# goroda/GPEXP

Measured on AMD Instinct MI355X. Metric: GP-fit+IVAR-eval points/s at N=32768 d=8 (wall-time in ms_per_step); value = (N+M)/t_step, SURVEY 8d's N/t_fit and M/t_IVAR are points_per_s_fit / points_per_s_ivar right behind it, higher is better.
Workload: dtype f64; 1 GPU; C4: N=32768 d=8 Matern-5/2 (rho=0.5,s=1,noise=0.1) kfill+potrf+potrs+logdet+IVAR over M=32768 MC points; N=32768, d=8, M=32768, kernel=matern52, seed=32768, parallelism=1 GPU

## Files before the change

### gpexp_amd/_lib.py

```python
import ctypes as C
import os

import numpy as np

_HERE = os.path.dirname(os.path.abspath(__file__))
LIB_PATH = os.path.join(_HERE, "libgpx_hip.so")

c_i64 = C.c_int64
c_dp = C.POINTER(C.c_double)
c_ip = C.POINTER(c_i64)
c_vp = C.c_void_p

_SIGS = {
    "gpx_abi_version": (C.c_int, []),
    "gpx_last_error": (C.c_char_p, []),
    "gpx_create": (C.c_int, [C.c_int, C.POINTER(c_vp)]),
    "gpx_destroy": (C.c_int, [c_vp]),
    "gpx_sync": (C.c_int, [c_vp]),
    "gpx_trim": (C.c_int, [c_vp]),
    "gpx_device_info": (C.c_int, [c_vp, C.c_char_p, C.c_int, C.POINTER(C.c_int), c_ip, C.POINTER(C.c_int)]),
    "gpx_mat_from_host": (C.c_int, [c_vp, c_dp, c_i64, c_i64, C.c_int, C.POINTER(c_vp)]),
    "gpx_mat_alloc": (C.c_int, [c_vp, c_i64, c_i64, C.c_int, C.POINTER(c_vp)]),
    "gpx_mat_free": (C.c_int, [c_vp, c_vp]),
    "gpx_mat_clone": (C.c_int, [c_vp, c_vp, C.POINTER(c_vp)]),
# ... 95 lines not shown
    "gpx_points_set_box": (C.c_int, [c_vp, c_vp, c_dp, c_dp, C.c_int]),
    "gpx_dist2_panel_pack": (C.c_int, [c_vp, c_vp, c_i64, c_i64, c_i64, c_i64, c_vp, c_i64, c_i64]),
    "gpx_dist2_diag_pack": (C.c_int, [c_vp, c_vp, c_i64, c_i64, c_i64, c_vp, c_i64, c_i64]),
    "gpx_dist2_update": (C.c_int, [c_vp, c_vp, c_i64, c_i64, c_i64, c_i64, c_vp, c_i64, c_i64, c_i64, c_i64]),
    "gpx_dist2_update_multi": (C.c_int, [c_vp, c_vp, c_i64, c_i64, c_i64, c_i64, c_i64, C.c_int, C.c_int, C.c_int, C.c_int, c_i64,
                                         C.c_int, C.POINTER(c_vp), c_ip, C.c_int]),
    "gpx_dist2_pack_rows": (C.c_int, [c_vp, c_vp, c_i64, c_i64, c_i64, c_vp, c_i64, c_i64, c_i64, c_i64]),
    "gpx_dist2_pack_diag": (C.c_int, [c_vp, c_vp, c_i64, c_i64, c_i64, c_vp, c_i64]),
    "gpx_program_run": (C.c_int, [c_vp, c_ip, c_i64, c_ip, c_i64, c_dp]),
    "gpx_program_capture": (C.c_int, [c_vp, c_ip, c_i64, c_ip, c_i64, C.POINTER(c_vp)]),
    "gpx_graph_launch": (C.c_int, [c_vp, c_vp, c_dp, c_ip]),
    "gpx_graph_free": (C.c_int, [c_vp, c_vp]),
    "gpx_dist2_unpack_rows": (C.c_int, [c_vp, c_vp, c_i64, c_i64, c_i64, c_i64, c_vp, c_i64, c_i64, c_i64]),
    "gpx_dist2_unpack_diag": (C.c_int, [c_vp, c_vp, c_i64, c_i64, c_i64, c_vp, c_i64]),
    "gpx_dist2_unpack_diag_at": (C.c_int, [c_vp, c_vp, c_i64, c_i64, c_i64, c_vp, c_i64, c_i64]),
    "gpx_dist2_trsv_diag": (C.c_int, [c_vp, c_vp, c_i64, c_i64, c_i64, c_vp, c_i64, C.c_int]),
    "gpx_dist2_gemv": (C.c_int, [c_vp, c_vp, c_i64, c_i64, c_i64, c_i64, c_vp, c_i64, c_vp, c_i64, C.c_int]),
    "gpx_dist2_logdet_acc": (C.c_int, [c_vp, c_vp, c_i64, c_i64, c_i64, c_i64, c_vp]),
    "gpx_stream_select": (C.c_int, [c_vp, C.c_int]),
    "gpx_event_record": (C.c_int, [c_vp, C.c_int]),
    "gpx_event_wait": (C.c_int, [c_vp, C.c_int]),
    "gpx_dist_finish": (C.c_int, [c_vp, c_vp]),
    "gpx_ivar_grad": (C.c_int, [c_vp, C.c_int, C.c_int, c_dp, C.c_int, c_vp, c_vp, c_vp, c_dp, c_dp]),
    "gpx_ivar_grad_w": (C.c_int, [c_vp, C.c_int, C.c_int, c_dp, C.c_int, c_vp, c_vp, c_vp, c_dp, c_vp, c_dp]),
    "gpx_ivar_grad_rows": (C.c_int, [c_vp, C.c_int, C.c_int, c_dp, C.c_int, c_vp, c_vp, c_vp, c_vp, c_i64, c_dp]),
    "gpx_var_grad": (C.c_int, [c_vp, C.c_int, C.c_int, c_dp, C.c_int, c_vp, c_vp, c_vp, c_dp, c_dp, c_dp, c_dp]),
    "gpx_var_grad_newpt": (C.c_int, [c_vp, C.c_int, C.c_int, c_dp, C.c_int, c_vp, c_vp, c_vp, c_dp]),
    "gpx_fitc_var_grad": (C.c_int, [c_vp, c_vp, C.c_int, C.c_int, c_dp, C.c_int, c_vp, c_vp, c_dp, c_dp, c_dp, c_dp]),
    "gpx_fitc_var_grad_newpt": (C.c_int, [c_vp, c_vp, C.c_int, C.c_int, c_dp, C.c_int, c_vp, c_vp, c_dp]),
    "gpx_profile_enable": (C.c_int, [c_vp, C.c_int]),
    "gpx_profile_reset": (C.c_int, [c_vp]),
    "gpx_profile_get": (C.c_int, [c_vp, C.c_int, c_ip, c_dp, c_dp, c_dp]),
    "gpx_dbg_gemm": (C.c_int, [c_vp, c_vp, c_vp, c_vp, C.c_int, C.c_int, C.c_int]),
    "gpx_dbg_gemm_tri": (C.c_int, [c_vp, c_vp, c_vp, c_vp, C.c_int, C.c_int, C.c_int]),
    "gpx_dbg_gemm_ksplit": (C.c_int, [c_vp, c_vp, c_vp, c_vp, C.c_int, C.c_int]),
    "gpx_dbg_kfill_plan": (C.c_int, [c_vp, C.c_int, C.c_int, c_dp, C.c_int, c_vp, c_vp, C.POINTER(C.c_int), c_dp]),
    "gpx_dbg_colreduce_plan": (C.c_int, [c_i64, c_i64, C.POINTER(c_i64), C.POINTER(c_i64)]),
    "gpx_dbg_panel_bcast_plan": (C.c_int, [C.c_int, C.c_int, c_i64, C.c_int, C.POINTER(c_i64), C.POINTER(C.c_int),
                                           C.POINTER(c_i64), c_i64, C.POINTER(c_i64)]),
    "gpx_dbg_guard_violations": (c_i64, [c_vp]),
    "gpx_dbg_guard_selftest": (C.c_int, [c_vp]),
    "gpx_dbg_spin": (C.c_int, [c_vp, C.c_int]),
    "gpx_dbg_spin_us": (C.c_int, [c_vp, c_i64]),
    "gpx_dbg_stamp": (C.c_int, [c_vp, C.c_int]),
    "gpx_dbg_spin_until": (C.c_int, [c_vp, C.c_int, c_i64]),
    "gpx_dbg_event_elapsed": (C.c_int, [c_vp, C.c_int, C.c_int, c_dp]),
    "gpx_dbg_leaf_stamps": (C.c_int, [c_vp, c_vp, C.c_int, C.POINTER(c_i64)]),
}

_lib = None


def load():
    global _lib
    if _lib is not None:
        return _lib
    path = os.environ.get("GPX_LIB_PATH", LIB_PATH)
    if not os.path.exists(path):
        raise ImportError(
            "gpexp_amd: %s not found - the HIP library is required (no CPU fallback). "
            "Build it with `make -C gpexp_amd/csrc` or __graft_entry__.build()." % path)
    lib = C.CDLL(path)
    for name, (res, args) in _SIGS.items():
        fn = getattr(lib, name)
        fn.restype = res
        fn.argtypes = args
# ... 41 lines not shown
```

### gpexp_amd/csrc/api.hip

```cpp
#include "gpx_internal.h"
#include <stdarg.h>
#include <stdio.h>
#include <string.h>
#include <math.h>
#include <stdlib.h>

static thread_local char g_err[1024] = "";

void gpx_set_error(const char* fmt, ...) {
  va_list ap;
  va_start(ap, fmt);
  vsnprintf(g_err, sizeof(g_err), fmt, ap);
  va_end(ap);
}

static constexpr int64_t GUARD = 4096;

int gpx_dev_alloc(gpx_ctx* ctx, int64_t bytes, void** out) {
  if (bytes <= 0) bytes = 8;
  bytes = gpx_round_up(bytes, 256);
  const int64_t key = bytes + (ctx->guard ? 2 * GUARD : 0);
  void* base = nullptr;
  auto it = ctx->pool.find(key);
  if (it != ctx->pool.end()) {
// ... 1383 lines not shown
  KParams kp;
  GPX_TRY(gpx_make_kparams(kind, d, hyp, nhyp, &kp));
  GPX_TRY(gpx_kparams_sets(ctx, &kp, X, Z));
  *exact = kp.exact;
  for (int k = 0; k < d; ++k) center[k] = kp.center[k];
  return 0;
}

int gpx_dbg_gemm_ksplit(gpx_ctx* ctx, const gpx_mat* A, const gpx_mat* B, gpx_mat* C, int mode, int parts) {
  GPX_ARG(ctx && A && B && C && mode >= 0 && mode <= 3 && parts > 0, "bad argument");
  const int64_t m = C->prows, n = C->pcols, k = A->pcols;
  GPX_ARG(A->prows == m && B->prows == n && B->pcols == k, "operand shapes");
  void* P;
  const int64_t pb = (int64_t)parts * m * n * 8;
  GPX_TRY(gpx_dev_alloc(ctx, pb, &P));
  int r = mode <= 1 ? launch_gemm_ksplit(ctx, A->p, A->ld, B->p, B->ld, C->p, C->ld, m, n, k, mode == 1, parts, (double*)P)
                    : launch_gemm_ksplit_small(ctx, A->p, A->ld, B->p, B->ld, C->p, C->ld, m, n, k, mode == 3, parts, (double*)P);
  (void)hipStreamSynchronize(ctx->stream);
  gpx_dev_release(ctx, P, pb);
  return r;
}

int gpx_dbg_gemm(gpx_ctx* ctx, const gpx_mat* A, const gpx_mat* B, gpx_mat* C, int bt, int accumulate, int lower) {
  GPX_ARG(ctx && A && B && C, "NULL argument");
  const int64_t m = C->prows, n = C->pcols, k = A->pcols;
  GPX_ARG(A->prows == m, "A rows");
  GPX_ARG(bt ? (B->prows == n && B->pcols == k) : (B->prows == k && B->pcols == n), "B shape");
  GPX_TRY(launch_gemm(ctx, A->p, A->ld, B->p, B->ld, C->p, C->ld, m, n, k, bt != 0, accumulate != 0,
                      lower != 0));
  GPX_HIP(hipStreamSynchronize(ctx->stream));
  return 0;
}

}
```

### gpexp_amd/csrc/chol.hip

```cpp
#include "gpx_internal.h"
#include <math.h>
#include <stdlib.h>
#include <stddef.h>

namespace {

constexpr int NB = GPX_TILE;
constexpr int LS = NB + 1;

typedef double d4 __attribute__((ext_vector_type(4)));

__device__ __forceinline__ double readlane_d(double v, int srclane) {
  int lo = __builtin_amdgcn_readlane(__double2loint(v), srclane);
  int hi = __builtin_amdgcn_readlane(__double2hiint(v), srclane);
  return __hiloint2double(hi, lo);
}

constexpr int LB = 16;
constexpr int TS17 = LB + 1;
constexpr int BSZ = LB * TS17;
constexpr int LEAF_CB = LB * LB + 64 + LB;

__device__ __forceinline__ constexpr int sb_off(int I, int J) { return (I * (I + 1) / 2 + J) * BSZ; }

// ... 1166 lines not shown

int chol_binv_ensure(gpx_ctx* ctx, gpx_mat* Lm) {
  const int64_t n = Lm->prows, ib = potrs_block(n);
  if (Lm->binv && Lm->binv_ib == ib) return 0;
  const int64_t nblk = (n + ib - 1) / ib;
  const int64_t bytes = chol_binv_elems(n) * 8;
  if (Lm->binv && Lm->binv_bytes != bytes) {
    gpx_dev_release(ctx, Lm->binv, Lm->binv_bytes);
    Lm->binv = nullptr;
  }
  if (!Lm->binv) {
    void* p;
    GPX_TRY(gpx_dev_alloc(ctx, bytes, &p));
    Lm->binv = (double*)p;
    Lm->binv_bytes = bytes;
  }
  void* pt;
  GPX_TRY(gpx_dev_alloc(ctx, nblk * ib * ib * 8, &pt));
  int r = binv_build_range(ctx, Lm->p, Lm->ld, Lm->aux, Lm->binv, ib, n, (double*)pt);
  if (r == 0) r = chol_binv_finish(ctx, Lm, ib);
  (void)hipStreamSynchronize(ctx->stream);
  gpx_dev_release(ctx, pt, nblk * ib * ib * 8);
  if (r != 0) Lm->binv_ib = 0;
  return r;
}

struct PotrsPlan {
  const double* L;
  int64_t ld, n, ib, nblk;
  int64_t sib;
  const double* binv;
  const double* binvT;
  double* part;
};
static inline int64_t blk_off(const PotrsPlan& P, int64_t b) { return b * P.ib < P.n ? b * P.ib : P.n; }
static inline const double* blk_inv(const PotrsPlan& P, const double* base, int64_t b) {
  const int64_t row = b * P.ib, sb = row / P.sib, within = row - sb * P.sib;
  return base + sb * P.sib * P.sib + within * P.sib + within;
}

static int potrs_fwd(gpx_ctx* ctx, const PotrsPlan& P, int64_t b0, int64_t b1, double* rhs, double* x) {
  if (b1 - b0 == 1) {
    const int64_t o = blk_off(P, b0), sz = blk_off(P, b0 + 1) - o;
    hipLaunchKernelGGL(binv_gemv_kernel, dim3((unsigned)((sz + 3) / 4)), dim3(256), 0, ctx->stream, blk_inv(P, P.binv, b0),
                       P.sib, sz, rhs + o, x + o, 1);
    return 0;
  }
  const int64_t mid = (b0 + b1) / 2;
  GPX_TRY(potrs_fwd(ctx, P, b0, mid, rhs, x));
  const int64_t r0 = blk_off(P, mid), r1 = blk_off(P, b1), c0 = blk_off(P, b0);
  int64_t wg = (r1 - r0 + 3) / 4;
  if (wg > 4096) wg = 4096;
  hipLaunchKernelGGL(gemv_sub_kernel, dim3((unsigned)wg), dim3(256), 0, ctx->stream, P.L + r0 * P.ld + c0, P.ld, r1 - r0, r0 - c0,
                     x + c0, rhs + r0);
  return potrs_fwd(ctx, P, mid, b1, rhs, x);
}

static int potrs_bwd(gpx_ctx* ctx, const PotrsPlan& P, int64_t b0, int64_t b1, double* rhs, double* z) {
  if (b1 - b0 == 1) {
    const int64_t o = blk_off(P, b0), sz = blk_off(P, b0 + 1) - o;
    hipLaunchKernelGGL(binv_gemv_kernel, dim3((unsigned)((sz + 3) / 4)), dim3(256), 0, ctx->stream, blk_inv(P, P.binvT, b0),
                       P.sib, sz, rhs + o, z + o, 0);
    return 0;
  }
  const int64_t mid = (b0 + b1) / 2;
  GPX_TRY(potrs_bwd(ctx, P, mid, b1, rhs, z));
  const int64_t r0 = blk_off(P, mid), r1 = blk_off(P, b1), c0 = blk_off(P, b0);
  GPX_TRY(launch_colreduce(ctx, P.L + r0 * P.ld + c0, P.ld, r1 - r0, r0 - c0, z + r0, rhs + c0, P.part, 1));
  return potrs_bwd(ctx, P, b0, mid, rhs, z);
}

static int trsm_left_oop_rec(gpx_ctx* ctx, const PotrsPlan& P, int64_t b0, int64_t b1, double* B, int64_t ldb, double* W,
                             int64_t ldw, int64_t m) {
  if (b1 - b0 == 1) {
    const int64_t o = blk_off(P, b0), sz = blk_off(P, b0 + 1) - o;
    return launch_gemm_tri(ctx, blk_inv(P, P.binv, b0), P.sib, B + o * ldb, ldb, W + o * ldw, ldw, sz, m, sz, false, false,
                           false, 1);
  }
  const int64_t mid = (b0 + b1) / 2;
  GPX_TRY(trsm_left_oop_rec(ctx, P, b0, mid, B, ldb, W, ldw, m));
  const int64_t r0 = blk_off(P, mid), r1 = blk_off(P, b1), c0 = blk_off(P, b0);
  GPX_TRY(launch_gemm(ctx, P.L + r0 * P.ld + c0, P.ld, W + c0 * ldw, ldw, B + r0 * ldb, ldb, r1 - r0, m, r0 - c0, false, true,
                      false));
  return trsm_left_oop_rec(ctx, P, mid, b1, B, ldb, W, ldw, m);
}

int chol_trsm_left_oop(gpx_ctx* ctx, gpx_mat* Lm, double* B, int64_t ldb, double* W, int64_t ldw, int64_t m) {
  GPX_ARG(Lm && Lm->factored && Lm->aux && B && W && B != W, "trsm: matrix has not been factored / bad buffers");
  if (m == 0) return 0;
  GPX_TRY(chol_binv_ensure(ctx, Lm));
  PotrsPlan P;
  P.L = Lm->p;
  P.ld = Lm->ld;
  P.n = Lm->prows;
  P.sib = Lm->binv_ib;
  P.ib = P.sib < 1024 ? P.sib : 1024;
  P.nblk = (P.n + P.ib - 1) / P.ib;
  P.binv = Lm->binv;
  P.binvT = nullptr;
  P.part = nullptr;
  return trsm_left_oop_rec(ctx, P, 0, P.nblk, B, ldb, W, ldw, m);
}

int chol_trsm_left_group(gpx_ctx* ctx, const double* Lg, int64_t ld, const double* invd, int64_t w, int64_t below, int64_t ib,
                         double* B, int64_t ldb, int64_t m, double* inv, double* tmp, double* W, int64_t ldw) {
  GPX_ARG(Lg && invd && B && inv && tmp && W && W != B && w > 0 && w % NB == 0 && ib >= NB && ib % NB == 0, "trsm group: bad arguments");
  if (m == 0) return 0;
  GPX_TRY(binv_build_range(ctx, Lg, ld, invd, inv, ib, w, tmp));
  PotrsPlan P;
  P.L = Lg;
  P.ld = ld;
  P.n = w;
  P.ib = P.sib = ib;
  P.nblk = (w + ib - 1) / ib;
  P.binv = inv;
  P.binvT = nullptr;
  P.part = nullptr;
  GPX_TRY(trsm_left_oop_rec(ctx, P, 0, P.nblk, B, ldb, W, ldw, m));
  if (below > 0) GPX_TRY(launch_gemm(ctx, Lg + w * ld, ld, W, ldw, B + w * ldb, ldb, below, m, w, false, true, false));
  return gpx_copy2d(ctx, W, ldw, B, ldb, w, m);
}

int64_t chol_potrs_scratch_bytes(int64_t n) { return n * 8 + colreduce_partial_elems(n, n) * 8 + 64; }

int chol_potrs(gpx_ctx* ctx, gpx_mat* Lm, double* v, double* scratch) {
  GPX_ARG(Lm && Lm->factored && Lm->aux && v && scratch, "potrs: matrix has not been factored / NULL vector");
  GPX_ARG(Lm->ld % 2 == 0, "potrs: leading dimension must be even");
  GPX_TRY(chol_binv_ensure(ctx, Lm));
  PotrsPlan P;
  P.L = Lm->p;
  P.ld = Lm->ld;
  P.n = Lm->prows;
  P.ib = P.sib = Lm->binv_ib;
  P.nblk = (P.n + P.ib - 1) / P.ib;
// ... 53 lines not shown
```

### gpexp_amd/csrc/gemm_f64.hip

```cpp
#include "gpx_internal.h"
#include <stdlib.h>

namespace {

typedef double d4 __attribute__((ext_vector_type(4)));

constexpr int KB = 16;
constexpr int SA = KB + 1;

template <bool BT, int TE>
struct Smem {
  double a[2][TE * SA];
  double b[2][BT ? TE * SA : KB * (TE + 16)];
};

template <bool LOWER>
__device__ __forceinline__ bool tile_of(int sblk, int within, int tiles_m, int tiles_n, int sb_cols, int sb_shift,
                                        int* by, int* bx, int rot = 0) {
  const int sbm = (1 << sb_shift) - 1;
  int sr, sc;
  if (LOWER) {
    const int nsr = (tiles_m + sbm) >> sb_shift;
    const int noff = nsr * (nsr - 1) / 2;
    if (sblk < noff) {
// ... 7 lines not shown
  } else {
    sr = sblk / sb_cols;
    sc = sblk - sr * sb_cols;
    if (rot) {
      if ((8 % sb_cols) == 0)
        sc = (sc + (sblk >> 3)) % sb_cols;
      else if ((sb_cols & 7) == 0)
        sc = (sc + sr) % sb_cols;
    }
  }
  *by = (sr << sb_shift) + (within >> sb_shift);
  *bx = (sc << sb_shift) + (within & sbm);
  if (!LOWER && rot == 2) {
    *by = (sr << sb_shift) + (within & sbm);
    *bx = (sc << sb_shift) + (sbm - (within >> sb_shift));
  }
  if (!LOWER && rot == 4) {
    *by = (sr << sb_shift) + (sbm - (within >> sb_shift));
    *bx = (sc << sb_shift) + (within & sbm);
  }
  if (!LOWER && rot == 3) {
    *by = (sr << sb_shift) + (within & sbm);
    *bx = (sc << sb_shift) + (within >> sb_shift);
  }
  if (*by >= tiles_m || *bx >= tiles_n) return false;
  if (LOWER && *bx > *by) return false;
  return true;
}

struct NoSeg {
  static constexpr bool on = false;
};

template <bool BT, bool ACC, int TE, class SEGF = NoSeg>
__device__ __forceinline__ void gemm_tile(Smem<BT, TE>& sm, const double* A, int64_t lda, const double* B, int64_t ldb,
                                          double* C, int64_t ldc, int nk, int by, int bx, const SEGF& segf = SEGF()) {
  constexpr int SBN = TE + 16;
  constexpr int FI = TE / 32;
  constexpr int NL = TE / 32;
  constexpr int WS = TE / 2;
  constexpr int BKR = 512 / TE;
  constexpr int A_BUF = TE * SA;
  constexpr int B_BUF = BT ? TE * SA : KB * SBN;

  const int t = threadIdx.x;
  const int lane = t & 63, wave = t >> 6;
  const int wm = wave >> 1, wn = wave & 1;
  const int64_t m0 = (int64_t)by * TE, n0 = (int64_t)bx * TE;

  const int ar = t >> 3, ac = (t & 7) * 2;
  const int br = t / (TE / 2), bc = (t % (TE / 2)) * 2;
  const unsigned voff_a = (unsigned)((ar * lda + ac) * 8);
  const unsigned voff_b = BT ? (unsigned)((ar * ldb + ac) * 8) : (unsigned)((br * ldb + bc) * 8);
  const char* const Abase = reinterpret_cast<const char*>(A + m0 * lda);
  const char* const Bbase = reinterpret_cast<const char*>(BT ? (B + n0 * ldb) : (B + n0));
  const int64_t a_rs = 32 * lda * 8;
  const int64_t b_rs = (BT ? 32 * ldb : BKR * ldb) * 8;
  const int64_t a_ks = (int64_t)KB * 8;
  const int64_t b_ks = (BT ? (int64_t)KB : (int64_t)KB * ldb) * 8;

  double2 Pa0, Pa1, Pa2, Pa3, Pb0, Pb1, Pb2, Pb3;
  const int64_t b_rs2 = 2 * b_rs, b_rs3 = 3 * b_rs, a_rs2 = 2 * a_rs, a_rs3 = 3 * a_rs;
#define GPX_LD16(base_, voff_) (*reinterpret_cast<const double2*>((base_) + (voff_)))
#define GPX_GLOAD_AT(S_, ap_, bp_)                                                                    \
  do {                                                                                                \
    S_##a0 = GPX_LD16(ap_, voff_a);                                                                    \
    S_##a1 = GPX_LD16(ap_ + a_rs, voff_a);                                                             \
    if (NL == 4) {                                                                                    \
      S_##a2 = GPX_LD16(ap_ + a_rs2, voff_a);                                                          \
// ... 140 lines not shown
      GPX_MFMAS(1);
      GPX_MFMAS(2);
      GPX_PIN();
      GPX_SSTORE(P, buf ^ 1);
      __syncthreads();
      GPX_PIN();
      GPX_FRAGS(buf ^ 1, 0, 0);
      GPX_FRAGS(buf ^ 1, 1, 1);
      GPX_FRAGS(buf ^ 1, 2, 2);
      GPX_PIN();
      GPX_MFMAS(3);
      GPX_FRAGS(buf ^ 1, 3, 3);
    }
    }
    GPX_MFMAS(0);
    GPX_MFMAS(1);
    GPX_MFMAS(2);
    GPX_MFMAS(3);
#undef GPX_STEP
#undef GPX_FRAGS
#undef GPX_MFMAS
#undef GPX_PIN
#undef GPX_PIN_ALL
  }
#undef GPX_GLOAD
#undef GPX_GLOAD_AT
#undef GPX_LD16
#undef GPX_SSTORE
#undef GPX_ST2
#undef GPX_STB
#undef GPX_COMPUTE

  double* Cw = C + (m0 + wm * WS + fk) * ldc + n0 + wn * WS + fr;
#pragma unroll
  for (int i = 0; i < FI; ++i)
#pragma unroll
    for (int v = 0; v < 4; ++v) {
      double* cp = Cw + (int64_t)(i * 16 + 4 * v) * ldc;
      if (ACC) {
        double cv[FI];
#pragma unroll
        for (int j = 0; j < FI; ++j) cv[j] = cp[j * 16];
#pragma unroll
        for (int j = 0; j < FI; ++j) cp[j * 16] = cv[j] - acc[i][j][v];
      } else {
#pragma unroll
        for (int j = 0; j < FI; ++j) cp[j * 16] = acc[i][j][v];
      }
    }
}

template <bool BT, bool ACC, bool LOWER, int TE, int TRI>
__global__ __launch_bounds__(256, 2) void gemm_f64_kernel(const double* A, int64_t lda, const double* B, int64_t ldb,
                                                          double* C, int64_t ldc, int nk, int tiles_m, int tiles_n,
                                                          int sb_cols, int sb_shift, int main_wgs, int tail_m0,
                                                          int tail_tn) {
  constexpr int tri = TRI;
  __shared__ Smem<BT, TE> sm;
  if (TE == 64 && tail_tn < 0) __builtin_amdgcn_s_setprio(3);
  const int w = blockIdx.x;
  if (TE == 128 && w >= main_wgs) {
    const int wt = w - main_wgs;
    const int by = wt / tail_tn, bx = wt - by * tail_tn;
    if (LOWER && 64 * bx > tail_m0 + 64 * by + 63) return;
    int64_t k0 = 0;
    if (tri == 3) k0 = tail_m0 + 64 * by;
    gemm_tile<BT, ACC, 64>(reinterpret_cast<Smem<BT, 64>&>(sm), A + (int64_t)tail_m0 * lda + k0, lda, B + k0, ldb,
                                 C + (int64_t)tail_m0 * ldc, ldc, nk - (int)(k0 / KB), by, bx);
    return;
  }
  const int xcd = w & 7, q = w >> 3;
  const int sbs2 = 2 * sb_shift;
  int by, bx;
  if (!tile_of<LOWER>((q >> sbs2) * 8 + xcd, q & ((1 << sbs2) - 1), tiles_m, tiles_n, sb_cols, sb_shift, &by, &bx,
                      tri == 2 ? 2 : (tri == 4 ? 3 : (tri == 1 ? 4 : 0))))
    return;
  int nkt = nk;
  if (tri == 1) nkt = min(nk, (by + 1) * (TE / KB));
  if (tri == 2) nkt = min(nk, (bx + 1) * (TE / KB));
  if (tri == 3) {
    const int64_t k0 = (int64_t)by * TE;
    A += k0;
    B += k0;
    nkt = nk - by * (TE / KB);
  }
  if (tri == 4) {
    const int64_t k0 = (int64_t)bx * TE;
    A += k0;
    B += k0 * ldb;
    nkt = nk - bx * (TE / KB);
  }
  gemm_tile<BT, ACC, TE>(sm, A, lda, B, ldb, C, ldc, nkt, by, bx);
}

template <bool BT, bool ACC>
__global__ __launch_bounds__(256, 2) void gemm_f64_batched_kernel(const double* A, int64_t lda, int64_t sa,
                                                                  const double* B, int64_t ldb, int64_t sb, double* C,
                                                                  int64_t ldc, int64_t sc, int nk, int tiles_n, int hiprio) {
  __shared__ Smem<BT, 64> sm;
  if (hiprio) __builtin_amdgcn_s_setprio(3);
  const int64_t b = blockIdx.y;
  const int by = blockIdx.x / tiles_n, bx = blockIdx.x - by * tiles_n;
  gemm_tile<BT, ACC, 64>(sm, A + b * sa, lda, B + b * sb, ldb, C + b * sc, ldc, nk, by, bx);
}

template <bool LOWER>
__global__ __launch_bounds__(256, 2) void gemm_f64_ksplit_kernel(const double* A, int64_t lda, const double* B, int64_t ldb,
                                                                 double* P, int64_t n, int64_t sp, int nk_slice, int parts,
                                                                 int tiles_m, int tiles_n, int sb_cols, int sb_shift) {
  __shared__ Smem<true, 128> sm;
  const int w = blockIdx.x, xcd = w & 7, q = w >> 3, sbs2 = 2 * sb_shift;
  const int job = (q >> sbs2) * 8 + xcd, within = q & ((1 << sbs2) - 1);
  int sb, slice;
  if (LOWER) {
    const int nsr = (tiles_m + (1 << sb_shift) - 1) >> sb_shift, noff = nsr * (nsr - 1) / 2;
    if (job < parts * noff) {
      slice = job / noff;
      sb = job - slice * noff;
    } else {
      const int jj = job - parts * noff;
      slice = jj / nsr;
      sb = noff + jj - slice * nsr;
    }
  } else {
    const int nsb = ((tiles_m + (1 << sb_shift) - 1) >> sb_shift) * sb_cols;
// ... 223 lines not shown
      gpx_set_error("gemm: triangular-operand mode %d is not instantiated for bt=%d accumulate=%d", tri, (int)bt, (int)accumulate);
      return -1;
    }
#undef GPX_GT
    GPX_HIP(hipGetLastError());
    return 0;
  }
#define GPX_K(BT_, ACC_, LOW_, TE_) GPX_KT(BT_, ACC_, LOW_, TE_, 0)
#define GPX_G(BT_, ACC_, LOW_)          \
  do {                                  \
    if (te == 64)                       \
      GPX_K(BT_, ACC_, LOW_, 64);       \
    else                                \
      GPX_K(BT_, ACC_, LOW_, 128);      \
  } while (0)
  if (bt) {
    if (accumulate) {
      if (lower) GPX_G(true, true, true); else GPX_G(true, true, false);
    } else {
      if (lower) GPX_G(true, false, true); else GPX_G(true, false, false);
    }
  } else {
    if (accumulate) {
      if (lower) GPX_G(false, true, true); else GPX_G(false, true, false);
    } else {
      if (lower) GPX_G(false, false, true); else GPX_G(false, false, false);
    }
  }
#undef GPX_G
#undef GPX_K
#undef GPX_KT
  GPX_HIP(hipGetLastError());
  return 0;
}

int launch_dist2_update(gpx_ctx* ctx, double* C, int64_t ldc, int64_t lr0, int64_t m, int64_t lc0, int64_t n, int64_t nb, int Pr,
                        int Pc, int pr, int pc, int64_t piece_stride, int64_t dsz, int nseg, const double* const* g,
                        const int64_t* ks, int below_diag) {
  if (m == 0 || n == 0 || nseg == 0) return 0;
  GPX_ARG(nseg > 0 && nseg <= GPX_SEG_MAX && Pr >= 1 && Pr <= GPX_MAX_PR && Pc >= 1, "dist2 update: too many segments / grid rows");
  GPX_ARG(m % 128 == 0 && n % 128 == 0 && nb % 128 == 0 && lr0 % nb == 0 && lc0 % nb == 0 && (ldc % 2) == 0, "dist2 update: alignment");
  Dist2Upd u;
  for (int s = 0; s < nseg; ++s) {
    u.g[s] = g[s];
    for (int p = 0; p < Pr; ++p) u.li0[s][p] = (int)(ks[s] + 1 <= p ? 0 : (ks[s] - p) / Pr + 1);
  }
  u.nseg = nseg;
  u.seg_nk = (int)(nb / KB);
  u.Pr = Pr; u.Pc = Pc; u.pr = pr; u.pc = pc;
  u.nb = (int)nb;
  u.gld = (int)gpx_g_ld(nb);
  u.li_first = (int)(lr0 / nb);
  u.lj_first = (int)(lc0 / nb);
  u.below_diag = below_diag;
  u.piece_stride = piece_stride;
  u.dsz = dsz;
  double tiles128 = 0.0;
  for (int64_t lj = lc0 / nb; lj * nb < lc0 + n; ++lj) {
    const int64_t J = lj * Pc + pc;
    const int64_t cw = (lc0 + n - lj * nb) < nb ? (lc0 + n - lj * nb) : nb;
    for (int64_t li = lr0 / nb; li * nb < lr0 + m; ++li) {
      const int64_t I = li * Pr + pr;
      if (I < J || (below_diag && I == J)) continue;
      const int64_t rh = (lr0 + m - li * nb) < nb ? (lr0 + m - li * nb) : nb;
      tiles128 += (double)(rh / 128) * (double)(cw / 128);
    }
// ... 51 lines not shown
```

### gpexp_amd/csrc/gpx_internal.h

```cpp
#pragma once
#include <hip/hip_runtime.h>
#include <stdint.h>
#include <stdlib.h>
#include <string>
#include <vector>
#include <map>
#include <memory>
#include <unordered_set>
#include "../../include/gpx.h"
#include "../../include/gpx_dist.h"
#include "../../include/gpx_debug.h"

#define GPX_TILE 128
#define GPX_MAXD GPX_MAX_DIM
#define GPX_NSTREAMS 6
#define GPX_SEG_MAX 8
#ifndef GPX_G_SKEW
#define GPX_G_SKEW 0
#endif
#define GPX_MAX_PR 4

void gpx_set_error(const char* fmt, ...);
#define GPX_HIP(call)                                                                   \
  do {                                                                                  \
// ... 128 lines not shown
  do {                            \
    if ((d_) <= 1) { CALL(1); }   \
    else if ((d_) <= 2) { CALL(2); } \
    else if ((d_) <= 4) { CALL(4); } \
    else if ((d_) <= 8) { CALL(8); } \
    else if ((d_) <= 16) { CALL(16); } \
    else { CALL(32); }            \
  } while (0)

extern "C" int64_t gpx_eval_chunk(int64_t np);

int launch_kfill(gpx_ctx* ctx, const KParams& kp, const double* A, int64_t na, const double* B, int64_t nb,
                 int symmetric, const double* d_nugget, int64_t nugget_len, double nugget_scalar,
                 double* out, int64_t prows, int64_t pcols, int64_t ld);
int launch_kfill_offset(gpx_ctx* ctx, const KParams& kp, const double* X, int64_t n, int64_t row_off, int64_t col_off,
                        const double* d_nugget, int64_t nugget_len, double nugget_scalar, double* out, int64_t prows,
                        int64_t pcols, int64_t ld);
int launch_kdiag(gpx_ctx* ctx, const KParams& kp, const double* Z, int64_t m, double* out);
int launch_kfill_cyclic(gpx_ctx* ctx, const KParams& kp, const double* X, int64_t n, const double* d_nugget,
                        int64_t nugget_len, double nugget_scalar, double* out, int64_t prows, int64_t pcols, int64_t ld,
                        int64_t nb, int Pr, int pr, int Pc, int pc);
int gpx_copy2d(gpx_ctx* ctx, const double* src, int64_t lds_, double* dst, int64_t ldd, int64_t rows, int64_t cols);
int gpx_copy2d_lower(gpx_ctx* ctx, const double* src, int64_t lds_, double* dst, int64_t ldd, int64_t n);
int launch_kfill_rows(gpx_ctx* ctx, const KParams& kp, const double* X, int64_t n, int64_t row0, const double* d_nugget,
                      int64_t nugget_len, double nugget_scalar, double* out, int64_t prows_band, int64_t pcols,
                      int64_t ld);

static inline int gpx_chain_prio(const gpx_ctx* ctx) { return ctx->stream == ctx->streams[1] ? 1 : 0; }
int launch_gemm(gpx_ctx* ctx, const double* A, int64_t lda, const double* B, int64_t ldb, double* C, int64_t ldc,
                int64_t m, int64_t n, int64_t k, bool bt, bool accumulate, bool lower);

int launch_gemm_tri(gpx_ctx* ctx, const double* A, int64_t lda, const double* B, int64_t ldb, double* C, int64_t ldc,
                    int64_t m, int64_t n, int64_t k, bool bt, bool accumulate, bool lower, int tri);
int launch_gemm_ksplit(gpx_ctx* ctx, const double* A, int64_t lda, const double* B, int64_t ldb, double* C, int64_t ldc,
                       int64_t m, int64_t n, int64_t k, bool lower, int64_t parts, double* P, bool assign = false);
int launch_gemm_ksplit_small(gpx_ctx* ctx, const double* A, int64_t lda, const double* B, int64_t ldb, double* C, int64_t ldc,
                             int64_t m, int64_t n, int64_t k, bool assign, int64_t parts, double* P);
int launch_gemm_batched(gpx_ctx* ctx, const double* A, int64_t lda, int64_t sa, const double* B, int64_t ldb, int64_t sb,
                        double* C, int64_t ldc, int64_t sc, int64_t m, int64_t n, int64_t k, bool bt, bool accumulate,
                        int64_t batch);

int launch_dist2_update(gpx_ctx* ctx, double* C, int64_t ldc, int64_t lr0, int64_t m, int64_t lc0, int64_t n, int64_t nb, int Pr,
                        int Pc, int pr, int pc, int64_t piece_stride, int64_t dsz, int nseg, const double* const* g,
                        const int64_t* ks, int below_diag);

int launch_leaf(gpx_ctx* ctx, double* A, int64_t ld, double* inv, int64_t base_index, int64_t n_valid);
int chol_potrf(gpx_ctx* ctx, double* A, int64_t ld, int64_t n, double* invd, int64_t n_valid);
int chol_potrf_nozero(gpx_ctx* ctx, double* A, int64_t ld, int64_t n, double* invd, int64_t base, int64_t n_valid);
int chol_trsm_right(gpx_ctx* ctx, const double* L, int64_t ldl, const double* invd, double* X, int64_t ldx,
                    int64_t m, int64_t n);
int chol_trsm_right_n(gpx_ctx* ctx, const double* L, int64_t ldl, const double* invd, double* X, int64_t ldx,
                      int64_t m, int64_t n);
int chol_trsm_left(gpx_ctx* ctx, const double* L, int64_t ldl, const double* invd, double* B, int64_t ldb,
                   int64_t n, int64_t m);
int chol_trsv(gpx_ctx* ctx, const double* L, int64_t ld, const double* invd, double* y, int64_t n, bool transposed);
int64_t chol_trsv_scratch_bytes(int64_t n);
int chol_trsv_with_scratch(gpx_ctx* ctx, const double* L, int64_t ld, const double* invd, double* y, int64_t n,
                           bool transposed, double* scratch);
int launch_logdet(gpx_ctx* ctx, const double* L, int64_t ld, int64_t n, double* d_out);
int chol_trtri(gpx_ctx* ctx, const gpx_mat* L, double* Linv, double* tmp);
int chol_binv_ensure(gpx_ctx* ctx, gpx_mat* L);
int chol_trsm_right_trailing(gpx_ctx* ctx, gpx_mat* L, int64_t r0, double* X, int64_t ldx, int64_t m, int transposed, double* T);
int chol_trsm_right_leading(gpx_ctx* ctx, gpx_mat* L, int64_t ncols, double* X, int64_t ldx, int64_t m, double* T, int64_t tcap);
int chol_trsm_right_n_leading(gpx_ctx* ctx, gpx_mat* L, int64_t ncols, double* X, int64_t ldx, int64_t m, double* T);
int chol_block_inverse(gpx_ctx* ctx, const double* D, int64_t ldd, const double* invd, double* inv, int64_t w, double* tmp);
int64_t chol_binv_order(int64_t n);
// ... 28 lines not shown
```

### gpexp_amd/device.py

```python
import ctypes as C
import atexit
import os

import numpy as np

from . import _lib
from ._lib import check, as_f64, dptr, c_vp, c_i64, GpxError

K_SE, K_MATERN32, K_MATERN52, K_MEHLER = 0, 1, 2, 3
PROF_CLASSES = ["kfill", "gemm", "leaf", "trsv", "reduce", "greedy", "comm", "kcross"]

_ctx = None


class Context:

    def __init__(self, device=None):
        self.lib = _lib.load()
        if device is None:
            device = int(os.environ.get("LOCAL_RANK", "0"))
        h = c_vp()
        rc = self.lib.gpx_create(int(device), C.byref(h))
        if rc != 0:
            raise RuntimeError("gpexp_amd needs an MI355X: " + self.lib.gpx_last_error().decode())
# ... 617 lines not shown

def var_grad(ctx, spec, L, X, Z, noise_deriv=None, eval_bias=None, dk_bias=None):
    out = np.empty((X.shape[0] * spec.d, Z.shape[0]))
    nd = as_f64(noise_deriv) if noise_deriv is not None else None
    eb = as_f64(eval_bias) if eval_bias is not None else None
    db = as_f64(dk_bias) if dk_bias is not None else None
    check(ctx.lib.gpx_var_grad(ctx.h, *spec.args(), L.h, X.h, Z.h, dptr(nd), dptr(eb), dptr(db), dptr(out)))
    return out


def var_grad_newpt(ctx, spec, L, X, Z):
    out = np.empty(Z.shape[0] * spec.d)
    check(ctx.lib.gpx_var_grad_newpt(ctx.h, *spec.args(), L.h, X.h, Z.h, dptr(out)))
    return out


def kfill_plan(ctx, spec, X, Z=None):
    ex = C.c_int()
    cen = np.zeros(spec.d)
    check(ctx.lib.gpx_dbg_kfill_plan(ctx.h, *spec.args(), X.h, Z.h if Z is not None else None, C.byref(ex), dptr(cen)))
    return bool(ex.value), cen


def dbg_gemm_tri(ctx, A, B, Cm, bt, accumulate, tri):
    check(ctx.lib.gpx_dbg_gemm_tri(ctx.h, A.h, B.h, Cm.h, int(bt), int(accumulate), int(tri)))


def dbg_gemm_ksplit(ctx, A, B, Cm, mode, parts):
    check(ctx.lib.gpx_dbg_gemm_ksplit(ctx.h, A.h, B.h, Cm.h, int(mode), int(parts)))


def dbg_gemm(ctx, A, B, Cm, bt, accumulate, lower=False):
    check(ctx.lib.gpx_dbg_gemm(ctx.h, A.h, B.h, Cm.h, int(bt), int(accumulate), int(lower)))
```

### include/gpx_debug.h

```cpp
#ifndef GPX_DEBUG_H
#define GPX_DEBUG_H
#include "gpx.h"
#ifdef __cplusplus
extern "C" {
#endif

int gpx_dbg_gemm(gpx_ctx* ctx, const gpx_mat* A, const gpx_mat* B, gpx_mat* C, int bt, int accumulate, int lower);
int gpx_dbg_gemm_tri(gpx_ctx* ctx, const gpx_mat* A, const gpx_mat* B, gpx_mat* C, int bt, int accumulate, int tri);
int gpx_dbg_gemm_ksplit(gpx_ctx* ctx, const gpx_mat* A, const gpx_mat* B, gpx_mat* C, int mode, int parts);
int gpx_dbg_spin(gpx_ctx* ctx, int ms);
int64_t gpx_dbg_guard_violations(gpx_ctx* ctx);
int gpx_dbg_guard_selftest(gpx_ctx* ctx);
int gpx_dbg_panel_bcast_plan(int W, int me, int64_t small_elems, int npieces, const int64_t* counts, const int* roots,
                             int64_t* ops, int64_t max_ops, int64_t* nops);
int gpx_dbg_colreduce_plan(int64_t rows, int64_t pcols, int64_t* nchunk, int64_t* bound_elems);
int gpx_dbg_kfill_plan(gpx_ctx* ctx, int kind, int d, const double* hyp, int nhyp, const gpx_mat* X, const gpx_mat* Z,
                       int* exact, double* center);

int gpx_dbg_spin_us(gpx_ctx* ctx, int64_t us);
int gpx_dbg_stamp(gpx_ctx* ctx, int slot);
int gpx_dbg_spin_until(gpx_ctx* ctx, int slot, int64_t us);
int gpx_dbg_event_elapsed(gpx_ctx* ctx, int id0, int id1, double* ms);

int gpx_dbg_leaf_stamps(gpx_ctx* ctx, gpx_mat* K, int fast, int64_t* out30);

#ifdef __cplusplus
}
#endif
#endif
```

Before: 97150 points/s.

## Use one-level Strassen for large GEMM updates in left out-of-place TRSM

Adds a one-level Strassen GEMM path for the trailing updates inside the recursive left triangular solve, used when the update block is large (at least 8192 rows and inner dimension, 4096 columns). Operand sums are formed by a small elementwise kernel. Five of the seven half-size products use a new dual-destination epilogue that subtracts into two C quadrants at once, so no temporary product buffers are needed. The aim is to cut roughly one eighth of the FP64 multiply work in the dominant solve GEMMs. The costs are extra scratch memory, extra memory traffic for the sums and the read-modify-write of two outputs, and slightly weaker numerical error bounds. It can be turned off with GPX_STRASSEN=0.

```diff
diff --git a/gpexp_amd/_lib.py b/gpexp_amd/_lib.py
--- a/gpexp_amd/_lib.py
+++ b/gpexp_amd/_lib.py
@@ -151,6 +151,7 @@
     "gpx_profile_reset": (C.c_int, [c_vp]),
     "gpx_profile_get": (C.c_int, [c_vp, C.c_int, c_ip, c_dp, c_dp, c_dp]),
     "gpx_dbg_gemm": (C.c_int, [c_vp, c_vp, c_vp, c_vp, C.c_int, C.c_int, C.c_int]),
+    "gpx_dbg_gemm_strassen": (C.c_int, [c_vp, c_vp, c_vp, c_vp]),
     "gpx_dbg_gemm_tri": (C.c_int, [c_vp, c_vp, c_vp, c_vp, C.c_int, C.c_int, C.c_int]),
     "gpx_dbg_gemm_ksplit": (C.c_int, [c_vp, c_vp, c_vp, c_vp, C.c_int, C.c_int]),
     "gpx_dbg_kfill_plan": (C.c_int, [c_vp, C.c_int, C.c_int, c_dp, C.c_int, c_vp, c_vp, C.POINTER(C.c_int), c_dp]),
diff --git a/gpexp_amd/csrc/api.hip b/gpexp_amd/csrc/api.hip
--- a/gpexp_amd/csrc/api.hip
+++ b/gpexp_amd/csrc/api.hip
@@ -1439,4 +1439,13 @@
   return 0;
 }
 
-}
+int gpx_dbg_gemm_strassen(gpx_ctx* ctx, const gpx_mat* A, const gpx_mat* B, gpx_mat* C) {
+  GPX_ARG(ctx && A && B && C, "NULL argument");
+  const int64_t m = C->prows, n = C->pcols, k = A->pcols;
+  GPX_ARG(A->prows == m && B->prows == k && B->pcols == n, "operand shapes");
+  GPX_TRY(launch_gemm_strassen(ctx, A->p, A->ld, B->p, B->ld, C->p, C->ld, m, n, k, nullptr, 0));
+  GPX_HIP(hipStreamSynchronize(ctx->stream));
+  return 0;
+}
+
+}
diff --git a/gpexp_amd/csrc/chol.hip b/gpexp_amd/csrc/chol.hip
--- a/gpexp_amd/csrc/chol.hip
+++ b/gpexp_amd/csrc/chol.hip
@@ -1222,6 +1222,9 @@
   const double* binv;
   const double* binvT;
   double* part;
+  bool strassen = false;
+  double* sscr = nullptr;
+  int64_t sscr_bytes = 0;
 };
 static inline int64_t blk_off(const PotrsPlan& P, int64_t b) { return b * P.ib < P.n ? b * P.ib : P.n; }
 static inline const double* blk_inv(const PotrsPlan& P, const double* base, int64_t b) {
@@ -1260,6 +1263,17 @@
   return potrs_bwd(ctx, P, b0, mid, rhs, z);
 }
 
+#ifndef GPX_STRASSEN_MIN_ROWS
+#define GPX_STRASSEN_MIN_ROWS 8192
+#endif
+#ifndef GPX_STRASSEN_MIN_COLS
+#define GPX_STRASSEN_MIN_COLS 4096
+#endif
+static inline bool strassen_gate(int64_t rows, int64_t cols, int64_t k) {
+  return rows >= GPX_STRASSEN_MIN_ROWS && k >= GPX_STRASSEN_MIN_ROWS && cols >= GPX_STRASSEN_MIN_COLS &&
+         gemm_strassen_scratch_bytes(rows, cols, k) > 0;
+}
+
 static int trsm_left_oop_rec(gpx_ctx* ctx, const PotrsPlan& P, int64_t b0, int64_t b1, double* B, int64_t ldb, double* W,
                              int64_t ldw, int64_t m) {
   if (b1 - b0 == 1) {
@@ -1270,8 +1284,12 @@
   const int64_t mid = (b0 + b1) / 2;
   GPX_TRY(trsm_left_oop_rec(ctx, P, b0, mid, B, ldb, W, ldw, m));
   const int64_t r0 = blk_off(P, mid), r1 = blk_off(P, b1), c0 = blk_off(P, b0);
-  GPX_TRY(launch_gemm(ctx, P.L + r0 * P.ld + c0, P.ld, W + c0 * ldw, ldw, B + r0 * ldb, ldb, r1 - r0, m, r0 - c0, false, true,
-                      false));
+  if (P.strassen && strassen_gate(r1 - r0, m, r0 - c0))
+    GPX_TRY(launch_gemm_strassen(ctx, P.L + r0 * P.ld + c0, P.ld, W + c0 * ldw, ldw, B + r0 * ldb, ldb, r1 - r0, m, r0 - c0,
+                                 P.sscr, P.sscr_bytes));
+  else
+    GPX_TRY(launch_gemm(ctx, P.L + r0 * P.ld + c0, P.ld, W + c0 * ldw, ldw, B + r0 * ldb, ldb, r1 - r0, m, r0 - c0, false,
+                        true, false));
   return trsm_left_oop_rec(ctx, P, mid, b1, B, ldb, W, ldw, m);
 }
 
@@ -1289,7 +1307,27 @@
   P.binv = Lm->binv;
   P.binvT = nullptr;
   P.part = nullptr;
-  return trsm_left_oop_rec(ctx, P, 0, P.nblk, B, ldb, W, ldw, m);
+  void* ps = nullptr;
+  int64_t sbytes = 0;
+  if (P.nblk >= 2 && env_i64("GPX_STRASSEN", 1) != 0) {
+    const int64_t r0 = blk_off(P, P.nblk / 2);
+    if (strassen_gate(P.n - r0, m, r0)) {
+      sbytes = gemm_strassen_scratch_bytes(P.n - r0, m, r0);
+      if (gpx_dev_alloc(ctx, sbytes, &ps) != 0) {
+        (void)hipGetLastError();
+        ps = nullptr;
+      }
+    }
+  }
+  P.strassen = ps != nullptr;
+  P.sscr = (double*)ps;
+  P.sscr_bytes = sbytes;
+  const int r = trsm_left_oop_rec(ctx, P, 0, P.nblk, B, ldb, W, ldw, m);
+  if (ps) {
+    (void)hipStreamSynchronize(ctx->stream);
+    gpx_dev_release(ctx, ps, sbytes);
+  }
+  return r;
 }
 
 int chol_trsm_left_group(gpx_ctx* ctx, const double* Lg, int64_t ld, const double* invd, int64_t w, int64_t below, int64_t ib,
diff --git a/gpexp_amd/csrc/gemm_f64.hip b/gpexp_amd/csrc/gemm_f64.hip
--- a/gpexp_amd/csrc/gemm_f64.hip
+++ b/gpexp_amd/csrc/gemm_f64.hip
@@ -63,9 +63,19 @@
   static constexpr bool on = false;
 };
 
-template <bool BT, bool ACC, int TE, class SEGF = NoSeg>
+struct NoDual {
+  static constexpr bool on = false;
+};
+struct Dual {
+  static constexpr bool on = true;
+  double* c2;
+  double s;
+};
+
+template <bool BT, bool ACC, int TE, class SEGF = NoSeg, class EPI = NoDual>
 __device__ __forceinline__ void gemm_tile(Smem<BT, TE>& sm, const double* A, int64_t lda, const double* B, int64_t ldb,
-                                          double* C, int64_t ldc, int nk, int by, int bx, const SEGF& segf = SEGF()) {
+                                          double* C, int64_t ldc, int nk, int by, int bx, const SEGF& segf = SEGF(),
+                                          const EPI& epi = EPI()) {
   constexpr int SBN = TE + 16;
   constexpr int FI = TE / 32;
   constexpr int NL = TE / 32;
@@ -272,6 +282,30 @@
 #undef GPX_COMPUTE
 
   double* Cw = C + (m0 + wm * WS + fk) * ldc + n0 + wn * WS + fr;
+  if constexpr (EPI::on) {
+    static_assert(ACC, "the two-destination epilogue accumulates");
+    double* Cw2 = epi.c2 + (m0 + wm * WS + fk) * ldc + n0 + wn * WS + fr;
+    const double s2 = epi.s;
+#pragma unroll
+    for (int i = 0; i < FI; ++i)
+#pragma unroll
+      for (int v = 0; v < 4; ++v) {
+        double* cp = Cw + (int64_t)(i * 16 + 4 * v) * ldc;
+        double* cq = Cw2 + (int64_t)(i * 16 + 4 * v) * ldc;
+        double cv[FI], cw[FI];
+#pragma unroll
+        for (int j = 0; j < FI; ++j) {
+          cv[j] = cp[j * 16];
+          cw[j] = cq[j * 16];
+        }
+#pragma unroll
+        for (int j = 0; j < FI; ++j) {
+          cp[j * 16] = cv[j] - acc[i][j][v];
+          cq[j * 16] = cw[j] - s2 * acc[i][j][v];
+        }
+      }
+    return;
+  }
 #pragma unroll
   for (int i = 0; i < FI; ++i)
 #pragma unroll
@@ -331,6 +365,49 @@
     nkt = nk - bx * (TE / KB);
   }
   gemm_tile<BT, ACC, TE>(sm, A, lda, B, ldb, C, ldc, nkt, by, bx);
+}
+
+template <int TE>
+__global__ __launch_bounds__(256, 2) void gemm_f64_dual_kernel(const double* A, int64_t lda, const double* B, int64_t ldb,
+                                                               double* C, double* C2, double s, int64_t ldc, int nk,
+                                                               int tiles_m, int tiles_n, int sb_cols, int sb_shift) {
+  __shared__ Smem<false, TE> sm;
+  const int w = blockIdx.x;
+  const int xcd = w & 7, q = w >> 3;
+  const int sbs2 = 2 * sb_shift;
+  int by, bx;
+  if (!tile_of<false>((q >> sbs2) * 8 + xcd, q & ((1 << sbs2) - 1), tiles_m, tiles_n, sb_cols, sb_shift, &by, &bx, 0)) return;
+  gemm_tile<false, true, TE, NoSeg, Dual>(sm, A, lda, B, ldb, C, ldc, nk, by, bx, NoSeg(), Dual{C2, s});
+}
+
+template <bool BSIDE>
+__global__ __launch_bounds__(256) void strassen_sums_kernel(const double* __restrict__ X, int64_t ldx, int64_t hr, int64_t hc,
+                                                            double* __restrict__ S, int64_t lds, int64_t sstride) {
+  const int64_t j = ((int64_t)blockIdx.x * 256 + threadIdx.x) * 2;
+  if (j >= hc) return;
+  for (int64_t i = blockIdx.y; i < hr; i += gridDim.y) {
+    const double* x1 = X + i * ldx + j;
+    const double* x2 = X + (i + hr) * ldx + j;
+    const double2 x11 = *reinterpret_cast<const double2*>(x1);
+    const double2 x12 = *reinterpret_cast<const double2*>(x1 + hc);
+    const double2 x21 = *reinterpret_cast<const double2*>(x2);
+    const double2 x22 = *reinterpret_cast<const double2*>(x2 + hc);
+    double* o = S + i * lds + j;
+#define GPX_S2(k_, ex_, ey_) *reinterpret_cast<double2*>(o + (k_) * sstride) = make_double2(ex_, ey_)
+    GPX_S2(0, x11.x + x22.x, x11.y + x22.y);
+    if (BSIDE) {
+      GPX_S2(1, x12.x - x22.x, x12.y - x22.y);
+      GPX_S2(2, x21.x - x11.x, x21.y - x11.y);
+      GPX_S2(3, x11.x + x12.x, x11.y + x12.y);
+      GPX_S2(4, x21.x + x22.x, x21.y + x22.y);
+    } else {
+      GPX_S2(1, x21.x + x22.x, x21.y + x22.y);
+      GPX_S2(2, x11.x + x12.x, x11.y + x12.y);
+      GPX_S2(3, x21.x - x11.x, x21.y - x11.y);
+      GPX_S2(4, x12.x - x22.x, x12.y - x22.y);
+    }
+#undef GPX_S2
+  }
 }
 
 template <bool BT, bool ACC>
@@ -620,6 +697,84 @@
 #undef GPX_KT
   GPX_HIP(hipGetLastError());
   return 0;
+}
+
+static int launch_gemm_dual(gpx_ctx* ctx, const double* A, int64_t lda, const double* B, int64_t ldb, double* C1, double* C2,
+                            double s, int64_t ldc, int64_t m, int64_t n, int64_t k) {
+  GPX_ARG(m % 128 == 0 && n % 128 == 0 && k % KB == 0 && k > 0 && m > 0 && n > 0, "gemm: m,n must be multiples of 128 and k of 16");
+  GPX_ARG((lda % 2) == 0 && (ldb % 2) == 0, "gemm: leading dimensions must be even (16-byte loads)");
+  const double tiles128 = (double)(m / 128) * (double)(n / 128);
+  const int te = tiles128 < 1024.0 ? 64 : 128;
+  const Plan p = make_plan(m, n, false, te);
+  GPX_ARG(p.wgs < ((int64_t)1 << 31), "gemm: grid too large");
+  const int nk = (int)(k / KB);
+  ProfScope ps(ctx, GPX_PROF_GEMM, 2.0 * (double)m * (double)n * (double)k, 0.0);
+  if (te == 64)
+    hipLaunchKernelGGL(gemm_f64_dual_kernel<64>, dim3((unsigned)p.wgs), dim3(256), 0, ctx->stream, A, lda, B, ldb, C1, C2, s, ldc,
+                       nk, p.tm, p.tn, p.sbc, p.sb_shift);
+  else
+    hipLaunchKernelGGL(gemm_f64_dual_kernel<128>, dim3((unsigned)p.wgs), dim3(256), 0, ctx->stream, A, lda, B, ldb, C1, C2, s, ldc,
+                       nk, p.tm, p.tn, p.sbc, p.sb_shift);
+  GPX_HIP(hipGetLastError());
+  return 0;
+}
+
+static inline bool strassen_shape_ok(int64_t m, int64_t n, int64_t k) {
+  return m > 0 && n > 0 && k > 0 && m % 256 == 0 && n % 256 == 0 && k % 32 == 0;
+}
+
+int64_t gemm_strassen_scratch_bytes(int64_t m, int64_t n, int64_t k) {
+  if (!strassen_shape_ok(m, n, k)) return 0;
+  const int64_t hm = m / 2, hn = n / 2, hk = k / 2;
+  return 5 * (hm * gpx_skew_ld(hk) + hk * gpx_skew_ld(hn)) * 8;
+}
+
+int launch_gemm_strassen(gpx_ctx* ctx, const double* A, int64_t lda, const double* B, int64_t ldb, double* C, int64_t ldc,
+                         int64_t m, int64_t n, int64_t k, double* scratch, int64_t scratch_bytes) {
+  const int64_t need = gemm_strassen_scratch_bytes(m, n, k);
+  if (need == 0 || (lda % 2) != 0 || (ldb % 2) != 0 || C == A || C == B)
+    return launch_gemm(ctx, A, lda, B, ldb, C, ldc, m, n, k, false, true, false);
+  void* own = nullptr;
+  if (!scratch || scratch_bytes < need) {
+    if (gpx_dev_alloc(ctx, need, &own) != 0) {
+      (void)hipGetLastError();
+      return launch_gemm(ctx, A, lda, B, ldb, C, ldc, m, n, k, false, true, false);
+    }
+    scratch = (double*)own;
+  }
+  const int64_t hm = m / 2, hn = n / 2, hk = k / 2, lsa = gpx_skew_ld(hk), lsb = gpx_skew_ld(hn);
+  const int64_t sa = hm * lsa, sb = hk * lsb;
+  double* const S = scratch;
+  double* const T = scratch + 5 * sa;
+  int r = 0;
+  do {
+    {
+      ProfScope ps(ctx, GPX_PROF_REDUCE, 5.0 * (double)hm * hk + 5.0 * (double)hk * hn, 72.0 * ((double)hm * hk + (double)hk * hn));
+      hipLaunchKernelGGL(strassen_sums_kernel<false>, dim3((unsigned)((hk / 2 + 255) / 256), (unsigned)(hm < 65535 ? hm : 65535)),
+                         dim3(256), 0, ctx->stream, A, lda, hm, hk, S, lsa, sa);
+      hipLaunchKernelGGL(strassen_sums_kernel<true>, dim3((unsigned)((hn / 2 + 255) / 256), (unsigned)(hk < 65535 ? hk : 65535)),
+                         dim3(256), 0, ctx->stream, B, ldb, hk, hn, T, lsb, sb);
+      if (hipGetLastError() != hipSuccess) {
+        gpx_set_error("strassen: operand-sum launch failed");
+        r = -2;
+        break;
+      }
+    }
+    const double *A11 = A, *A22 = A + hm * lda + hk, *B11 = B, *B22 = B + hk * ldb + hn;
+    double *C11 = C, *C12 = C + hn, *C21 = C + hm * ldc, *C22 = C + hm * ldc + hn;
+    if ((r = launch_gemm_dual(ctx, S, lsa, T, lsb, C11, C22, 1.0, ldc, hm, hn, hk)) != 0) break;
+    if ((r = launch_gemm_dual(ctx, S + sa, lsa, B11, ldb, C21, C22, -1.0, ldc, hm, hn, hk)) != 0) break;
+    if ((r = launch_gemm_dual(ctx, A11, lda, T + sb, lsb, C12, C22, 1.0, ldc, hm, hn, hk)) != 0) break;
+    if ((r = launch_gemm_dual(ctx, A22, lda, T + 2 * sb, lsb, C11, C21, 1.0, ldc, hm, hn, hk)) != 0) break;
+    if ((r = launch_gemm_dual(ctx, S + 2 * sa, lsa, B22, ldb, C12, C11, -1.0, ldc, hm, hn, hk)) != 0) break;
+    if ((r = launch_gemm(ctx, S + 3 * sa, lsa, T + 3 * sb, lsb, C22, ldc, hm, hn, hk, false, true, false)) != 0) break;
+    if ((r = launch_gemm(ctx, S + 4 * sa, lsa, T + 4 * sb, lsb, C11, ldc, hm, hn, hk, false, true, false)) != 0) break;
+  } while (0);
+  if (own) {
+    (void)hipStreamSynchronize(ctx->stream);
+    gpx_dev_release(ctx, own, need);
+  }
+  return r;
 }
 
 int launch_dist2_update(gpx_ctx* ctx, double* C, int64_t ldc, int64_t lr0, int64_t m, int64_t lc0, int64_t n, int64_t nb, int Pr,
diff --git a/gpexp_amd/csrc/gpx_internal.h b/gpexp_amd/csrc/gpx_internal.h
--- a/gpexp_amd/csrc/gpx_internal.h
+++ b/gpexp_amd/csrc/gpx_internal.h
@@ -184,6 +184,9 @@
 
 int launch_gemm_tri(gpx_ctx* ctx, const double* A, int64_t lda, const double* B, int64_t ldb, double* C, int64_t ldc,
                     int64_t m, int64_t n, int64_t k, bool bt, bool accumulate, bool lower, int tri);
+int64_t gemm_strassen_scratch_bytes(int64_t m, int64_t n, int64_t k);
+int launch_gemm_strassen(gpx_ctx* ctx, const double* A, int64_t lda, const double* B, int64_t ldb, double* C, int64_t ldc,
+                         int64_t m, int64_t n, int64_t k, double* scratch, int64_t scratch_bytes);
 int launch_gemm_ksplit(gpx_ctx* ctx, const double* A, int64_t lda, const double* B, int64_t ldb, double* C, int64_t ldc,
                        int64_t m, int64_t n, int64_t k, bool lower, int64_t parts, double* P, bool assign = false);
 int launch_gemm_ksplit_small(gpx_ctx* ctx, const double* A, int64_t lda, const double* B, int64_t ldb, double* C, int64_t ldc,
diff --git a/gpexp_amd/device.py b/gpexp_amd/device.py
--- a/gpexp_amd/device.py
+++ b/gpexp_amd/device.py
@@ -673,3 +673,7 @@
 
 def dbg_gemm(ctx, A, B, Cm, bt, accumulate, lower=False):
     check(ctx.lib.gpx_dbg_gemm(ctx.h, A.h, B.h, Cm.h, int(bt), int(accumulate), int(lower)))
+
+
+def dbg_gemm_strassen(ctx, A, B, Cm):
+    check(ctx.lib.gpx_dbg_gemm_strassen(ctx.h, A.h, B.h, Cm.h))
diff --git a/include/gpx_debug.h b/include/gpx_debug.h
--- a/include/gpx_debug.h
+++ b/include/gpx_debug.h
@@ -8,6 +8,7 @@
 int gpx_dbg_gemm(gpx_ctx* ctx, const gpx_mat* A, const gpx_mat* B, gpx_mat* C, int bt, int accumulate, int lower);
 int gpx_dbg_gemm_tri(gpx_ctx* ctx, const gpx_mat* A, const gpx_mat* B, gpx_mat* C, int bt, int accumulate, int tri);
 int gpx_dbg_gemm_ksplit(gpx_ctx* ctx, const gpx_mat* A, const gpx_mat* B, gpx_mat* C, int mode, int parts);
+int gpx_dbg_gemm_strassen(gpx_ctx* ctx, const gpx_mat* A, const gpx_mat* B, gpx_mat* C);
 int gpx_dbg_spin(gpx_ctx* ctx, int ms);
 int64_t gpx_dbg_guard_violations(gpx_ctx* ctx);
 int gpx_dbg_guard_selftest(gpx_ctx* ctx);
```

Result: faster. 102,600 points/s, median of 6 (+5.6%).
